# multimodallearning/DG-TTA

Measured on AMD Instinct MI355X. Metric: TTA-epochs/sec per GPU on 128^3 patch; Dice delta vs reference, higher is better.
Workload: dtype fp16

## Files before the change

### dg_tta_amd/_lib.py

```python
import ctypes as C
import os
from pathlib import Path

LIB_PATH = Path(__file__).resolve().parent / "libdgtta_hip.so"

_c_float_p = C.POINTER(C.c_float)
P, I, I64, U64, F, SZ = C.c_void_p, C.c_int, C.c_int64, C.c_uint64, C.c_float, C.c_size_t

SIGNATURES = {
    "dgtta_version": (I, []),
    "dgtta_last_error": (C.c_char_p, []),
    "dgtta_reload_env": (I, []),
    "dgtta_mind3d_ws_bytes": (SZ, [I, I, I, I]),
    "dgtta_mind3d_fwd": (I, [P, P, F, I, C.POINTER(F), I, P, I, I, I, P, SZ, I, I, I, I, P]),
    "dgtta_mind3d_noise_fill": (I, [P, U64, U64, I, I, I, I, I, P]),
    "dgtta_mind3d_fwd_seeded": (I, [P, U64, U64, I, F, I, C.POINTER(F), I, P, I, I, I, P, SZ, I, I, I, I, P]),
    "dgtta_gin_ws_bytes": (SZ, [I, I, I, I]),
    "dgtta_gin_chain_fwd": (I, [P, P, C.POINTER(I), C.POINTER(P), C.POINTER(P), P, P, SZ, I, I, I, I, P]),
    "dgtta_affine_warp3d_fwd": (I, [P, P, P, I, I, I, I, I, I, I, I, I, I, I, I, I, I, P, P]),
    "dgtta_affine_warp3d_bwd": (I, [P, P, P, I, I, I, I, I, I, I, I, I, I, I, I, I, P]),
    "dgtta_rf_field_ws_bytes": (SZ, [I, I, I, I]),
    "dgtta_rf_field_fwd": (I, [P, P, P, SZ, I, I, I, I, I, I, I, I, P]),
    "dgtta_diffeo_fields_ws_bytes": (SZ, [I, I, I, I]),
    "dgtta_diffeo_fields": (I, [P, F, P, P, P, SZ, I, I, I, I, I, P]),
# ... 47 lines not shown
    "dgtta_conv3d_kwgrad_ws_bytes": (SZ, [I, I, I, I, I, I, I, I, I, I]),
    "dgtta_conv3d_wgrad": (I, [P, I, P, I, P, P, P, SZ, I, I, I, I, I, I, I, I, I, I, I, I, P]),
    "dgtta_convT3d_s_fwd_ws_bytes": (SZ, [I, I, I, I, I, I]),
    "dgtta_convT3d_s_fwd": (I, [P, I, P, P, P, I, P, SZ, I, I, I, I, I, I, I, I, I, I, P]),
    "dgtta_convT3d_s_bwd_ws_bytes": (SZ, [I, I, I, I, I, I, I, I, I]),
    "dgtta_convT3d_s_bwd": (I, [P, I, P, I, P, P, I, P, P, P, SZ, I, I, I, I, I, I, I, I, I, I, I, P]),
    "dgtta_seghead_fwd": (I, [P, I, P, P, P, I, P, I, I, I, I, I64, I, P]),
    "dgtta_seghead_bwd_ws_bytes": (SZ, [I, I, I, I64]),
    "dgtta_seghead_bwd": (I, [P, I, P, I, P, P, I, P, I, P, P, P, SZ, I, I, I64, I, I, P]),
    "dgtta_seghead_bwd_acc": (I, [P, I, P, I, P, P, I, P, I, P, P, P, SZ, I, I, I64, I, I, I, P]),
    "dgtta_seghead_warp_supported": (I, [P, I, I, I, I, I, I, I]),
    "dgtta_seghead_warp_bwd_ws_bytes": (SZ, [I, I, I, I, I, I]),
    "dgtta_seghead_warp_fwd": (I, [P, P, P, P, I, P, P, I, I, I, I, I, I, I, P]),
    "dgtta_seghead_warp_bwd": (I, [P, P, P, P, P, P, I, P, P, P, P, SZ, I, I, I, I, I, I, I, I, P]),
    "dgtta_seghead_warp_bwd_g16": (I, [P, P, P, P, P, P, I, P, P, P, P, SZ, I, I, I, I, I, I, I, I, P]),
    "dgtta_ncdhw_to_ndhwc": (I, [P, P, I, I, I64, I, I, P]),
    "dgtta_ndhwc_to_ncdhw": (I, [P, P, I, I, I64, I, I, P]),
    "dgtta_argmax_dice": (I, [P, I, I, P, P, P, I, I64, P]),
    "dgtta_resample_axis_ws_bytes": (SZ, [I64, I, I64, I]),
    "dgtta_resample_axis": (I, [P, P, P, SZ, I64, I, I, I64, I, P]),
    "dgtta_window_accumulate": (I, [P, P, P, P, I, I, I, I, I, I, I, I, I, I, P]),
    "dgtta_seghead_window_accumulate": (I, [P, P, P, P, P, P, I, I, I, I, I, I, I, I, I, I, I, I, P]),
    "dgtta_logits_chunk_f64": (I, [P, P, P, I, I, I, I, I, I, I, I, I, I, I, I, P]),
    "dgtta_window_accumulate_t": (I, [P, P, P, P, I, I, I, I, I, I, I, I, I, I, I, P]),
    "dgtta_seghead_window_accumulate_t": (I, [P, P, P, P, P, P, I, I, I, I, I, I, I, I, I, I, I, I, I, P]),
    "dgtta_argmax_rows": (I, [P, I, I, I64, P, P]),
    "dgtta_feature_window_accumulate": (I, [P, P, P, P, I, I, I, I, I, I, I, I, I, I, I, P]),
    "dgtta_feature_window_accumulate_norm": (I, [P, P, P, P, F, P, P, P, I, I, I, I, I, I, I, I, I, I, I, P]),
    "dgtta_feature_window_accumulate_multi": (I, [P, P, P, I, P, P, F, P, P, P, I, I, I, I, I, I, I, I, I, I, I, I, P]),
    "dgtta_feature_head_argmax": (I, [P, I64, P, P, P, I, I, I, I64, P, P]),
# ... 103 lines not shown
```

### dg_tta_amd/csrc/conv_api.h

```cpp
#pragma once
#include "common.h"

static inline bool dtype_ok(int dtype) { return dtype == DGTTA_F32 || dtype == DGTTA_BF16 || dtype == DGTTA_F16; }
static inline size_t esize(int dtype) { return dtype == DGTTA_F32 ? 4 : 2; }

static inline int conv_granule(int dtype) { return dtype == DGTTA_F32 ? 8 : 16; }
static inline size_t n32(int c) { return (size_t)(c + 31) / 32 * 32; }

static inline int out_dim(int i, int s, int k = 3) { return (i + 2 * (k / 2) - k) / s + 1; }

static inline int gs_blocks(int64_t total, int cap = 16384) {
  int64_t b = (total + 255) / 256;
  return (int)(b < cap ? (b > 0 ? b : 1) : cap);
}

static inline int reduce_blocks(int64_t V, int B) {
  int64_t b = cdiv64(V, 32);
  int64_t cap = 4096 / (B > 0 ? B : 1);
  if (cap < 128) cap = 128;
  if (cap > 2048) cap = 2048;
  return (int)(b < cap ? (b > 0 ? b : 1) : cap);
}

struct ConvProblem {
// ... 65 lines not shown

int conv3_wgrad_mfma(const ConvProblem &P, Src x, Src dy, float *dw_t, Region ws, int accumulate);
size_t conv3_wgrad_mfma_ws_bytes(int B, int Cin, int Cout, int D, int H, int W);
size_t conv3_wgrad_split_extra_bytes(int B, int Cin, int Cout, int D, int H, int W, int stride);
bool conv3_wgrad_blocked_ok(const ConvProblem &P);
size_t conva_wgrad_ws_bytes(int B, int Cin, int Cout, int D, int H, int W);
int conva_wgrad_mfma(const ConvProblem &P, Src x, Src dy, float *dw_t, Region ws, int accumulate);

int convT_wgrad_mfma(const ConvProblem &P, Src x, Src dout, float *dw_t, Region ws, int accumulate, Region bias_part, int *bias_units);
int convT_bias_finalize(const float *part, int units, int Cout, float *db, int accumulate, hipStream_t st);
size_t convT_wgrad_split_extra_bytes(int B, int Cin, int Cout, int Di, int Hi, int Wi);
int convTa_wgrad_mfma(const ConvProblem &P, Src x, Src dout, float *dw_t, Region ws, int accumulate);

size_t head_wgrad_mfma_ws_bytes(int Cin, int nsel, int64_t rows);
int head_wgrad_mfma(const void *x, int ldx, const float *dout, int lddo, float *dw_sel, void *ws, size_t ws_bytes, int Cin,
                    int nsel, int64_t rows, int accumulate, int dtype, hipStream_t st, bool have_d16);

int head_fwd_mfma(const void *x, int ldx, const float *w, const float *bias, const int *sel, int nsel, float *out, int ldo, int Cin,
                  int64_t rows, int dtype, hipStream_t st);
int head_dgrad_mfma(const float *dout, int lddo, const float *w, const int *sel, int nsel, void *dx, int lddx, int Cin, int64_t rows,
                    int accumulate_dx, int dtype, hipStream_t st);
int head_wgrad_rows_mfma(const void *x, int ldx, const float *dout, int lddo, float *part, int nsplit, int nsel, int Cin, int64_t rows,
                         int dtype, hipStream_t st);

int conv3_pack_weights_ref(const ConvProblem &P, const float *w_t, void *wf, void *wb);
int conv3_fwd_ref(const ConvProblem &P, Src x, const void *wf, const float *bias, Dst y);
int conv3_dgrad_ref(const ConvProblem &P, Src dy, const void *wb, Dst dx, int accumulate);
int conv3_wgrad_ref(const ConvProblem &P, Src x, Src dy, float *part, int nsplit, float *dw_t, int accumulate);
int convT_fwd_ref(const ConvProblem &P, Src x, const float *w_t, const float *bias, Dst out);
int convT_dgrad_ref(const ConvProblem &P, Src dout, const float *w_t, Dst dx);
int convT_wgrad_ref(const ConvProblem &P, Src x, Src dout, float *part, int nsplit, float *dw_t, int accumulate);
// ... 35 lines not shown
```

### dg_tta_amd/csrc/head_wgrad.hip

```cpp
#include "conv_wgrad_common.h"

namespace {
template <typename T16>
__global__ void f32_to_16_rows_kernel(const float *__restrict__ src, int lds_, unsigned short *__restrict__ dst, int C,
                                      int64_t rows) {
  const int64_t n = rows * C;
  for (int64_t i = (int64_t)blockIdx.x * blockDim.x + threadIdx.x; i < n; i += (int64_t)gridDim.x * blockDim.x)
    dst[i] = f32_to_16<T16>(src[(i / C) * lds_ + i % C]);
}
}

struct PWG {
  static constexpr int CHUNK = 128, NBUF = 4, LA = 2;
  static constexpr int X_B = CHUNK * 64, BUF_B = 2 * X_B;
  static constexpr int LDS_BYTES = NBUF * BUF_B;
};

template <typename T16>
__global__ __launch_bounds__(256, 2) void pointwise_wgrad_kernel(const bf16_t *__restrict__ x, int ldx,
                                                                 const unsigned short *__restrict__ d16, int nsel,
                                                                 float *__restrict__ partial, int64_t nchunks) {
  extern __shared__ __attribute__((aligned(16))) unsigned char smem[];
  const int tid = threadIdx.x, lane = tid & 63;
  const int wave = __builtin_amdgcn_readfirstlane(tid >> 6);
// ... 59 lines not shown
      if (g + j < G) s += v[j];
  }
  if (k < nsel && c < Cin) {
    float *o = dw + (int64_t)k * Cin + c;
    *o = accumulate ? *o + s : s;
  }
}

size_t head_wgrad_mfma_ws_bytes(int Cin, int nsel, int64_t rows) {
  if (rows <= 0 || rows % 128 || rows / 128 >= (1ll << 30)) return 0;
  const int D = (int)(rows / 128);
  return conv3_wgrad_mfma_ws_bytes(1, Cin, nsel, D, 4, 32) + align_up((size_t)rows * nsel * 2, 256);
}

int head_wgrad_mfma(const void *x, int ldx, const float *dout, int lddo, float *dw_sel, void *ws, size_t ws_bytes, int Cin,
                    int nsel, int64_t rows, int accumulate, int dtype, hipStream_t st, bool have_d16) {
  if (rows % 128 || rows / 128 >= (1ll << 30)) return DGTTA_ERR_UNSUPPORTED;
  const int D = (int)(rows / 128);
  if (ws_bytes < head_wgrad_mfma_ws_bytes(Cin, nsel, rows)) return DGTTA_ERR_UNSUPPORTED;
  Taps real;
  for (int t = 0; t < 27; ++t) real.wt[t] = -1;
  real.wt[13] = 0;
  RealTaps reals;
  const WgradClasses wc = wgrad_single_class(1u << 13, real, &reals);
  const WgradOut out{dw_sel, Cin, 1, 0, accumulate};
  WgradLaunch L{x, dense_view(1, D, 4, 32, ldx), dout, dense_view(1, D, 4, 32, lddo), 1, Cin, nsel, dtype, ws, ws_bytes, st};
  if (dtype == DGTTA_F32) return wgrad_launch_classes(L, out, wc, reals);
  if (dtype == DGTTA_BF16 || dtype == DGTTA_F16) {
    const size_t cbytes = align_up((size_t)rows * nsel * 2, 256);
    unsigned short *d16 = (unsigned short *)ws;
    if (!have_d16) {
      if (dtype == DGTTA_BF16)
        hipLaunchKernelGGL(f32_to_16_rows_kernel<bf16_t>, dim3(2048), dim3(256), 0, st, dout, lddo, d16, nsel, rows);
      else
        hipLaunchKernelGGL(f32_to_16_rows_kernel<f16_t>, dim3(2048), dim3(256), 0, st, dout, lddo, d16, nsel, rows);
      DG_CHECK_LAUNCH("f32_to_16_rows_kernel");
    }
    const int G = 512;
    if (Cin == 32 && ldx >= 32 && ldx % 8 == 0 && nsel % 8 == 0 && nsel <= 32 && !((uintptr_t)x & 15) &&
        ws_bytes - cbytes >= (size_t)G * 1024 * sizeof(float) && dgtta_switches().wgrad_tr != '0') {
      float *partial = reinterpret_cast<float *>((char *)ws + cbytes);
      const int64_t nchunks = rows / PWG::CHUNK;
      const int g = (int)(nchunks < G ? nchunks : G);
      static DynLdsOnce once_b, once_h;
      if (dtype == DGTTA_BF16) {
// ... 23 lines not shown
```

### dg_tta_amd/csrc/instnorm.hip

```cpp
#include "conv_api.h"
#include "gfx950.h"

namespace {

template <typename T, int MODE>
__global__ __launch_bounds__(256) void chan_reduce_kernel(const T *__restrict__ y, int ldy, const T *__restrict__ gz,
                                                          int ldgz, const float *__restrict__ mean_rstd,
                                                          const float *__restrict__ gamma,
                                                          const float *__restrict__ beta, float slope,
                                                          double *__restrict__ partial, int C, int64_t V) {
  __shared__ float red[2][256];
  const int b = blockIdx.y;
  int CL = 1;
  while (CL < C && CL < 64) CL <<= 1;
  const int RG = 256 / CL;
  const int cl = threadIdx.x % CL, rg = threadIdx.x / CL;
  const int64_t rows_per_blk = cdiv64(V, gridDim.x);
  const int64_t r0 = (int64_t)blockIdx.x * rows_per_blk, r1 = (r0 + rows_per_blk < V) ? r0 + rows_per_blk : V;
  for (int c0 = 0; c0 < C; c0 += CL) {
    const int c = c0 + cl;
    float s0 = 0.f, s1 = 0.f;
    if (c < C) {
      float mu = 0.f, rs = 0.f, ga = 0.f, be = 0.f;
      if (MODE == 1) {
// ... 370 lines not shown
    float g = ld_f<T>(gz + row * ldgz + c);
    g = a > 0.f ? g : g * slope;
    st_f<T>(dy + row * lddy + c, (ga * rs) * ((g - c12[bc * 2]) - xh * c12[bc * 2 + 1]));
  }
}

__global__ void bias_finalize_kernel(const double *__restrict__ partial, int nblk, int B, int C, float *__restrict__ db,
                                     int accumulate) {
  const int c = blockIdx.x;
  double s = 0.0;
  for (int k = threadIdx.x; k < B * nblk; k += 64) s += partial[(((int64_t)k * C) + c) * 2];
  s = wave_sum_d(s);
  if (threadIdx.x == 0) db[c] = accumulate ? db[c] + (float)s : (float)s;
}

}

__global__ void set_header_kernel(long long *hdr, long long v) { hdr[0] = v; }

int conv_stats_ref(const void *y, int ldy, void *stats, int B, int C, int64_t V, int dtype, hipStream_t st) {
  const int nblk = reduce_blocks(V, B);
  hipLaunchKernelGGL(set_header_kernel, dim3(1), dim3(1), 0, st, (long long *)stats, (long long)nblk);
  DISPATCH_T(dtype, hipLaunchKernelGGL((chan_reduce_kernel<T, 0>), dim3(nblk, B), dim3(256), 0, st, (const T *)y, ldy,
                                       (const T *)nullptr, 0, nullptr, nullptr, nullptr, 0.f, (double *)stats + 32,
                                       C, V));
  DG_CHECK_LAUNCH("chan_reduce_kernel<0>");
  return DGTTA_OK;
}

size_t conv_bias_grad_ws_bytes(int B, int C, int64_t V) {
// ... 99 lines not shown
                                        float *dbeta, void *ws, size_t ws_bytes, int B, int C, int64_t V, float slope,
                                        int accumulate, int dtype, void *stream) {
  return instnorm_bwd_impl(gz, ldgz, y, ldy, gamma, beta, mean_rstd, dy, lddy, dgamma, dbeta, nullptr, ws, ws_bytes, B, C, V,
                           slope, accumulate, dtype, stream, "instnorm_lrelu_bwd");
}

extern "C" int dgtta_instnorm_lrelu_bwd_gstats(const void *gz, int ldgz, const void *y, int ldy, const float *gamma,
                                               const float *beta, const float *mean_rstd, void *dy, int lddy,
                                               float *dgamma, float *dbeta, const void *gstats, void *ws, size_t ws_bytes,
                                               int B, int C, int64_t V, float slope, int accumulate, int dtype,
                                               void *stream) {
  DG_REQUIRE(gstats, DGTTA_ERR_BADARG, "instnorm_lrelu_bwd_gstats: null statistics");
  return instnorm_bwd_impl(gz, ldgz, y, ldy, gamma, beta, mean_rstd, dy, lddy, dgamma, dbeta, gstats, ws, ws_bytes, B, C, V,
                           slope, accumulate, dtype, stream, "instnorm_lrelu_bwd_gstats");
}
```

### dg_tta_amd/csrc/warp.hip

```cpp
#include "conv_api.h"
#include "gfx950.h"
#include "sampler.h"
#include <limits.h>

namespace {


__device__ __forceinline__ Sample sample_from_base(const float *th, float x, float y, float z, int Ds, int Hs, int Ws,
                                                   int algebra, int pad_mode);

__device__ __forceinline__ Sample sample_pos(const float *th, int d, int h, int w, int Dd, int Hd, int Wd, int Ds,
                                             int Hs, int Ws, int algebra, int pad_mode) {
  return sample_from_base(th, base_coord(w, Wd), base_coord(h, Hd), base_coord(d, Dd), Ds, Hs, Ws, algebra, pad_mode);
}

__device__ __forceinline__ Sample sample_from_base(const float *th, float x, float y, float z, int Ds, int Hs, int Ws,
                                                   int algebra, int pad_mode) {
  float gx = __builtin_fmaf(th[2], z, __builtin_fmaf(th[1], y, th[0] * x)) + th[3];
  float gy = __builtin_fmaf(th[6], z, __builtin_fmaf(th[5], y, th[4] * x)) + th[7];
  float gz = __builtin_fmaf(th[10], z, __builtin_fmaf(th[9], y, th[8] * x)) + th[11];
  if (algebra) {
    gx = (gx - x) + x;
    gy = (gy - y) + y;
    gz = (gz - z) + z;
// ... 506 lines not shown
    }
    f32x4_t a0 = {0.f, 0.f, 0.f, 0.f}, a1 = {0.f, 0.f, 0.f, 0.f};
#pragma unroll
    for (int s = 0; s < 8; s += 2) {
      a0 = __builtin_amdgcn_mfma_f32_16x16x4f32(wa[s], zbl[s], a0, 0, 0, 0);
      a1 = __builtin_amdgcn_mfma_f32_16x16x4f32(wa[s + 1], zbl[s + 1], a1, 0, 0, 0);
    }
    if (live && 4 * g < nsel) {
      float *op = out + ((int64_t)b * V + ((int64_t)d * H + h) * W + wv) * nsel + 4 * g;
      *reinterpret_cast<float4 *>(op) = make_float4((a0[0] + a1[0]) + b4[0] * wsum, (a0[1] + a1[1]) + b4[1] * wsum,
                                                    (a0[2] + a1[2]) + b4[2] * wsum, (a0[3] + a1[3]) + b4[3] * wsum);
    }
  }
}

template <typename T, bool G16 = false>
__global__ __launch_bounds__(256, 6) void head_warp_bwd_kernel(const void *__restrict__ gdst_, const float *__restrict__ theta,
                                                            const float *__restrict__ w, const int *__restrict__ sel,
                                                            int nsel, T *__restrict__ gz, unsigned short *__restrict__ d16,
                                                            double *__restrict__ bias_partial, int D, int H, int W,
                                                            int algebra, int gx, int gy) {
  __shared__ float sw[HW_NS * HW_CIN];
  __shared__ InvMap s_im;
  __shared__ float sred[4][HW_NS];
  const float *gdst = (const float *)gdst_;
  const unsigned short *gdst16 = (const unsigned short *)gdst_;
  for (int i = threadIdx.x; i < HW_NS * HW_CIN; i += 256) {
    const int k = i / HW_CIN;
    sw[i] = k < nsel ? w[(int64_t)(sel ? sel[k] : k) * HW_CIN + i % HW_CIN] : 0.f;
  }
  const int64_t V = (int64_t)D * H * W;
  const int tilesZ = (D + 3) >> 2;
  const int tile = (int)blockIdx.x;
  const int bx = tile % gx, by = (tile / gx) % gy, bz = tile / (gx * gy);
  const int b = bz / tilesZ;
  const int x = bx * 16 + (threadIdx.x & 15), y = by * 4 + ((threadIdx.x >> 4) & 3), zc_ = (bz % tilesZ) * 4 + (threadIdx.x >> 6);
  const float *th = theta + b * 12;
  if (threadIdx.x == 0) s_im = inverse_map(th, D, H, W, D, H, W, algebra);
  __syncthreads();
  const InvMap im = s_im;
  float acc[HW_NS];
#pragma unroll
  for (int q = 0; q < HW_NS; ++q) acc[q] = 0.f;
  const bool inside = x < W && y < H && zc_ < D;
// ... 79 lines not shown
              }
            }
          }
        }
      }
    }
  }
  if (inside) {
    const int64_t u = (int64_t)b * V + ((int64_t)zc_ * H + y) * W + x;
    unsigned short *dp = d16 + u * nsel;
#pragma unroll
    for (int q = 0; q < HW_NS; q += 4)
      if (q < nsel) *reinterpret_cast<uint2 *>(dp + q) = make_uint2(pack2_16<T>(acc[q], acc[q + 1]), pack2_16<T>(acc[q + 2], acc[q + 3]));
    T *gp = gz + u * HW_CIN;
#pragma unroll
    for (int qt = 0; qt < 4; ++qt) {
      float o[8] = {0.f, 0.f, 0.f, 0.f, 0.f, 0.f, 0.f, 0.f};
#pragma unroll
      for (int k = 0; k < HW_NS; ++k) {
        const float4 w0 = *reinterpret_cast<const float4 *>(sw + k * HW_CIN + qt * 8);
        const float4 w1 = *reinterpret_cast<const float4 *>(sw + k * HW_CIN + qt * 8 + 4);
        o[0] = __builtin_fmaf(acc[k], w0.x, o[0]);
        o[1] = __builtin_fmaf(acc[k], w0.y, o[1]);
        o[2] = __builtin_fmaf(acc[k], w0.z, o[2]);
        o[3] = __builtin_fmaf(acc[k], w0.w, o[3]);
        o[4] = __builtin_fmaf(acc[k], w1.x, o[4]);
        o[5] = __builtin_fmaf(acc[k], w1.y, o[5]);
        o[6] = __builtin_fmaf(acc[k], w1.z, o[6]);
        o[7] = __builtin_fmaf(acc[k], w1.w, o[7]);
      }
      *reinterpret_cast<uint4 *>(reinterpret_cast<unsigned short *>(gp) + qt * 8) = pack16<T>(o);
// ... 209 lines not shown
      hipLaunchKernelGGL((head_warp_fwd_mfma_kernel<f16_t>), dim3((unsigned)nblk), dim3(256), 0, (hipStream_t)stream,
                         (const f16_t *)z, theta, w, bias, sel, nsel, out, D, H, W, tta_grid_algebra, gx, gy);
  } else if (dtype == DGTTA_BF16) {
    HWF_LAUNCH(bf16_t);
  } else {
    HWF_LAUNCH(f16_t);
  }
#undef HWF_LAUNCH
  DG_CHECK_LAUNCH("head_warp_fwd_kernel");
  return DGTTA_OK;
}

static int seghead_warp_bwd_impl(const void *z, const void *gout, int gout16, const float *theta, const float *h_theta,
                                 const float *w, const int *sel, int nsel, void *gz, float *dw_sel, float *db_sel, void *ws,
                                 size_t ws_bytes, int B, int Cin, int D, int H, int W, int tta_grid_algebra, int accumulate,
                                 int dtype, void *stream) {
  DG_REQUIRE(z && gout && theta && h_theta && w && gz && ws, DGTTA_ERR_BADARG, "seghead_warp_bwd: null pointer");
  DG_REQUIRE(B > 0 && B <= 16 && D > 0 && H > 0 && W > 0, DGTTA_ERR_BADARG, "seghead_warp_bwd: bad dims");
  DG_REQUIRE(head_warp_shape_ok(Cin, nsel, dtype), DGTTA_ERR_UNSUPPORTED, "seghead_warp_bwd: unsupported shape / dtype");
  DG_REQUIRE(!dw_sel || head_warp_wgrad_ok(nsel), DGTTA_ERR_UNSUPPORTED,
             "seghead_warp_bwd: the weight gradient needs 8 or 16 selected classes (nsel %d; use the unfused path)", nsel);
  DG_REQUIRE(((uintptr_t)gout & 15) == 0 && ((uintptr_t)gz & 15) == 0, DGTTA_ERR_BADARG, "seghead_warp_bwd: unaligned operand");
  const size_t need = dgtta_seghead_warp_bwd_ws_bytes(B, Cin, nsel, D, H, W);
  DG_REQUIRE(need > 0, DGTTA_ERR_UNSUPPORTED, "seghead_warp_bwd: voxel count must be a multiple of 128");
  DG_REQUIRE(ws_bytes >= need, DGTTA_ERR_WORKSPACE, "seghead_warp_bwd: workspace too small");
  for (int b = 0; b < B; ++b)
    DG_REQUIRE(host_map_ok(h_theta + 12 * b, D, H, W), DGTTA_ERR_UNSUPPORTED,
               "seghead_warp_bwd: sample %d's map is singular or strongly minifying (use the unfused path)", b);
  hipStream_t st = (hipStream_t)stream;
  const int64_t rows = (int64_t)B * D * H * W;
  double *bias_partial = (double *)ws;
  void *ws_main = (char *)ws + head_warp_bias_region(B, D, H, W);
  const size_t main_bytes = ws_bytes - head_warp_bias_region(B, D, H, W);
  unsigned short *d16 = (unsigned short *)ws_main;
  const int gx = cdiv(W, 16), gy = cdiv(H, 4);
  const int64_t nblk = (int64_t)gx * gy * cdiv(D, 4) * B;
  DG_REQUIRE(nblk < (1ll << 31), DGTTA_ERR_UNSUPPORTED, "seghead_warp_bwd: too many tiles");
#define HWB_LAUNCH(T, G)                                                                                            \
  hipLaunchKernelGGL((head_warp_bwd_kernel<T, G>), dim3((unsigned)nblk), dim3(256), 0, st, gout, theta, w, sel, nsel, \
                     (T *)gz, d16, db_sel ? bias_partial : nullptr, D, H, W, tta_grid_algebra, gx, gy)
  if (dtype == DGTTA_BF16) {
    if (gout16) HWB_LAUNCH(bf16_t, true);
    else HWB_LAUNCH(bf16_t, false);
  } else {
    if (gout16) HWB_LAUNCH(f16_t, true);
    else HWB_LAUNCH(f16_t, false);
  }
#undef HWB_LAUNCH
  DG_CHECK_LAUNCH("head_warp_bwd_kernel");
  if (dw_sel) {
    const int rc = head_wgrad_mfma(z, Cin, nullptr, nsel, dw_sel, ws_main, main_bytes, Cin, nsel, rows, accumulate, dtype, st, true);
    DG_REQUIRE(rc == DGTTA_OK, rc, "seghead_warp_bwd: head weight gradient failed (%d)", rc);
  }
  if (db_sel) {
    hipLaunchKernelGGL(head_warp_bias_finalize_kernel, dim3(HW_NS), dim3(1024), 0, st, bias_partial, (int)nblk, nsel, db_sel,
                       accumulate);
    DG_CHECK_LAUNCH("head_warp_bias_finalize_kernel");
  }
  return DGTTA_OK;
}

extern "C" int dgtta_seghead_warp_bwd(const void *z, const float *gout, const float *theta, const float *h_theta,
                                      const float *w, const int *sel, int nsel, void *gz, float *dw_sel, float *db_sel,
                                      void *ws, size_t ws_bytes, int B, int Cin, int D, int H, int W, int tta_grid_algebra,
                                      int accumulate, int dtype, void *stream) {
  return seghead_warp_bwd_impl(z, gout, 0, theta, h_theta, w, sel, nsel, gz, dw_sel, db_sel, ws, ws_bytes, B, Cin, D, H, W,
                               tta_grid_algebra, accumulate, dtype, stream);
}

extern "C" int dgtta_seghead_warp_bwd_g16(const void *z, const void *gout16, const float *theta, const float *h_theta,
                                          const float *w, const int *sel, int nsel, void *gz, float *dw_sel, float *db_sel,
                                          void *ws, size_t ws_bytes, int B, int Cin, int D, int H, int W, int tta_grid_algebra,
                                          int accumulate, int dtype, void *stream) {
  return seghead_warp_bwd_impl(z, gout16, 1, theta, h_theta, w, sel, nsel, gz, dw_sel, db_sel, ws, ws_bytes, B, Cin, D, H, W,
                               tta_grid_algebra, accumulate, dtype, stream);
}
```

### dg_tta_amd/unet_exec.py

```python
import collections
import contextlib
import ctypes as C
import os

import torch

from . import _lib
from ._lib import check, ptr, stream_of
from ._state import state_of
from .ops import F32, F16, _ws, dtype_code

EPS, SLOPE = 1e-5, 1e-2


def _wgrad_on_side_stream():
    return os.environ.get("DGTTA_WGRAD_STREAM", "1") != "0"


def _pad(c, m):
    return (c + m - 1) // m * m


def _k3(k):
    return tuple(k) if isinstance(k, (tuple, list)) else (k, k, k)
# ... 444 lines not shown
    D, H, W = dims
    cin = head.in_channels
    assert gz.ld >= cin and z.ld >= cin
    g = gout.contiguous(memory_format=torch.channels_last_3d).float()
    need_hw = head.weight.requires_grad or head.bias.requires_grad
    dws = p.empty(nsel, cin, dtype=torch.float32) if need_hw else None
    dbs = p.empty(nsel, dtype=torch.float32) if need_hw else None
    nb = p.lib.dgtta_seghead_bwd_ws_bytes(p.B, cin, nsel, D * H * W)
    ws = p.ws.get(nb)
    check(p.lib.dgtta_seghead_bwd_acc(z.ptr, z.ld, ptr(g), nsel, ptr(head.weight), ptr(sel), nsel, gz.ptr, gz.ld, ptr(dws), ptr(dbs),
                                      ptr(ws), nb, p.B, cin, D * H * W, 0, 1, p.dt, p.st), "dgtta_seghead_bwd_acc")
    if need_hw:
        _scatter_head_grads(p, head, sel, dws, dbs)


def _head_backward(p, head, z, sel, nsel, fw, g16, gout, dims):
    lib, B, dt, st = p.lib, p.B, p.dt, p.st
    D, H, W = dims
    if g16 is not None and any(gout.stride()):
        gout = gout + g16.permute(0, 4, 1, 2, 3).float()
        g16 = None
    g = None if g16 is not None else gout.contiguous(memory_format=torch.channels_last_3d).float()
    cin = head.in_channels
    gz = p.empty(B, D, H, W, cin)
    need_hw = head.weight.requires_grad or head.bias.requires_grad
    dws = p.empty(nsel, cin, dtype=torch.float32) if need_hw else None
    dbs = p.empty(nsel, dtype=torch.float32) if need_hw else None
    if fw is not None:
        nb = lib.dgtta_seghead_warp_bwd_ws_bytes(B, cin, nsel, D, H, W)
        ws = p.ws.get(nb)
        assert g16 is None or (tuple(g16.shape) == (B, D, H, W, nsel) and g16.dtype == p.adt and g16.is_contiguous())
        bwd = lib.dgtta_seghead_warp_bwd if g16 is None else lib.dgtta_seghead_warp_bwd_g16
        check(bwd(z.ptr, ptr(g if g16 is None else g16), ptr(fw[0]), ptr(fw[1]), ptr(head.weight), ptr(sel), nsel, ptr(gz),
                  ptr(dws), ptr(dbs), ptr(ws), nb, B, cin, D, H, W, 1, 0, dt, st), bwd.__name__)
    else:
        nb = lib.dgtta_seghead_bwd_ws_bytes(B, cin, nsel, D * H * W)
        ws = p.ws.get(nb)
        check(lib.dgtta_seghead_bwd(z.ptr, z.ld, ptr(g), nsel, ptr(head.weight), ptr(sel), nsel, ptr(gz), cin, ptr(dws), ptr(dbs),
                                    ptr(ws), nb, B, cin, D * H * W, 0, dt, st), "dgtta_seghead_bwd")
    if need_hw:
        _scatter_head_grads(p, head, sel, dws, dbs)
    return _Rows(gz, gz.data_ptr(), cin)


def _norm_backward(p, blk, gz, gstats):
    lib, B, cout, v = p.lib, p.B, blk.cout, blk.vout
    norm = blk.mod.norm
    dy = p.empty(B, *blk.dout, cout)
    nb = lib.dgtta_instnorm_ws_bytes(B, cout, v)
    ws = p.ws.get(nb)
    dgam = p.gbuf(norm.weight) if norm.weight.requires_grad else torch.empty_like(norm.weight)
    dbet = p.gbuf(norm.bias) if norm.bias.requires_grad else torch.empty_like(norm.bias)
    if gstats is not None:
        check(lib.dgtta_instnorm_lrelu_bwd_gstats(gz.ptr, gz.ld, ptr(blk.y), cout, ptr(norm.weight), ptr(norm.bias), ptr(blk.mr),
                                                  ptr(dy), cout, ptr(dgam), ptr(dbet), ptr(gstats), ptr(ws), nb, B, cout, v,
                                                  SLOPE, p.acc, p.dt, p.st), "dgtta_instnorm_lrelu_bwd_gstats")
    else:
        check(lib.dgtta_instnorm_lrelu_bwd(gz.ptr, gz.ld, ptr(blk.y), cout, ptr(norm.weight), ptr(norm.bias), ptr(blk.mr), ptr(dy),
                                           cout, ptr(dgam), ptr(dbet), ptr(ws), nb, B, cout, v, SLOPE, p.acc, p.dt, p.st),
              "dgtta_instnorm_lrelu_bwd")
    return dy


def _weight_grad(p, blk, dy):
    conv = blk.mod.conv
    if not (conv.weight.requires_grad or conv.bias.requires_grad):
        return
    nb = blk.wgrad_ws_bytes(p)
# ... 122 lines not shown
```

### include/dgtta.h

```cpp
#ifndef DGTTA_H
#define DGTTA_H

#include <stddef.h>
#include <stdint.h>

#ifdef __cplusplus
extern "C" {
#endif

#define DGTTA_OK 0
#define DGTTA_ERR_BADARG (-1)
#define DGTTA_ERR_UNSUPPORTED (-2)
#define DGTTA_ERR_WORKSPACE (-3)
#define DGTTA_ERR_LAUNCH (-4)

#define DGTTA_F32 0
#define DGTTA_BF16 1
#define DGTTA_F16 2

#define DGTTA_PAD_ZEROS 0
#define DGTTA_PAD_BORDER 1
#define DGTTA_INTERP_LINEAR 0
#define DGTTA_INTERP_NEAREST 1

// ... 111 lines not shown
                             float *mean_rstd, void *z, int ldz, void *ws, size_t ws_bytes, int B, int C,
                             int64_t V, float eps, float slope, int dtype, void *stream);
int dgtta_instnorm_lrelu_bwd(const void *gz, int ldgz, const void *y, int ldy, const float *gamma,
                             const float *beta, const float *mean_rstd, void *dy, int lddy, float *dgamma,
                             float *dbeta, void *ws, size_t ws_bytes, int B, int C, int64_t V, float slope,
                             int accumulate, int dtype, void *stream);

int dgtta_conv3d_k3_dgrad_gstats(const void *dy, int lddy, const void *wpack, void *dx, int lddx, int B, int Cin, int Cout,
                                 int CinP, int CoutP, int Di, int Hi, int Wi, const void *y_prev, int ldy_prev,
                                 const float *mean_rstd_prev, const float *gamma_prev, const float *beta_prev, float slope,
                                 void *gstats, size_t gstats_bytes, int *h_produced, int dtype, int impl, void *stream);
int dgtta_instnorm_lrelu_bwd_gstats(const void *gz, int ldgz, const void *y, int ldy, const float *gamma, const float *beta,
                                    const float *mean_rstd, void *dy, int lddy, float *dgamma, float *dbeta,
                                    const void *gstats, void *ws, size_t ws_bytes, int B, int C, int64_t V, float slope,
                                    int accumulate, int dtype, void *stream);

size_t dgtta_convT3d_fwd_ws_bytes(int Cin, int Cout, int dtype);
int dgtta_convT3d_k2s2_fwd(const void *x, int ldx, const float *w_t, const float *bias, void *out, int ldo, void *ws,
                           size_t ws_bytes, int B, int Cin, int Cout, int Di, int Hi, int Wi, int dtype, int impl,
                           void *stream);
size_t dgtta_convT3d_bwd_ws_bytes(int B, int Cin, int Cout, int Di, int Hi, int Wi);
size_t dgtta_convT3d_bwd_split_ws_bytes(int B, int Cin, int Cout, int Di, int Hi, int Wi);
int dgtta_convT3d_k2s2_bwd(const void *x, int ldx, const void *dout, int lddo, const float *w_t, void *dx, int lddx,
                           float *dw_t, float *db, void *ws, size_t ws_bytes, int B, int Cin, int Cout, int Di,
                           int Hi, int Wi, int accumulate, int dtype, int impl, void *stream);

size_t dgtta_conv3d_kpacked_bytes(int kd, int CinP, int CoutP, int dtype);
int dgtta_conv3d_kpack_weights(const float *w_t, void *wpack, int kd, int kh, int kw, int Cin, int Cout, int CinP, int CoutP,
                               int dtype, void *stream);
int dgtta_conv3d_fwd(const void *x, int ldx, const void *wpack, const float *bias, void *y, int ldy, void *stats, int B, int Cin,
// ... 20 lines not shown
                      int B, int Cin, int64_t V, int accumulate, int dtype, void *stream);
int dgtta_seghead_bwd_acc(const void *x, int ldx, const float *dout, int lddo, const float *w, const int *sel,
                          int nsel, void *dx, int lddx, float *dw_sel, float *db_sel, void *ws, size_t ws_bytes,
                          int B, int Cin, int64_t V, int accumulate, int accumulate_dx, int dtype, void *stream);

int dgtta_seghead_warp_supported(const float *h_theta, int B, int Cin, int nsel, int D, int H, int W, int dtype);
size_t dgtta_seghead_warp_bwd_ws_bytes(int B, int Cin, int nsel, int D, int H, int W);
int dgtta_seghead_warp_fwd(const void *z, const float *w, const float *bias, const int *sel, int nsel, const float *theta,
                           float *out, int B, int Cin, int D, int H, int W, int tta_grid_algebra, int dtype, void *stream);
int dgtta_seghead_warp_bwd(const void *z, const float *gout, const float *theta, const float *h_theta, const float *w,
                           const int *sel, int nsel, void *gz, float *dw_sel, float *db_sel, void *ws, size_t ws_bytes, int B,
                           int Cin, int D, int H, int W, int tta_grid_algebra, int accumulate, int dtype, void *stream);
int dgtta_seghead_warp_bwd_g16(const void *z, const void *gout16, const float *theta, const float *h_theta, const float *w,
                               const int *sel, int nsel, void *gz, float *dw_sel, float *db_sel, void *ws, size_t ws_bytes, int B,
                               int Cin, int D, int H, int W, int tta_grid_algebra, int accumulate, int dtype, void *stream);

int dgtta_ncdhw_to_ndhwc(const float *src, void *dst, int B, int C, int64_t V, int ldc, int dtype, void *stream);
int dgtta_ndhwc_to_ncdhw(const void *src, float *dst, int B, int C, int64_t V, int ldc, int dtype, void *stream);

int dgtta_argmax_dice(const float *logits, int ldc, int C, const int64_t *labels, int64_t *argmax_out,
                      int64_t *counts, int B, int64_t V, void *stream);

int dgtta_window_accumulate(const float *patch, const float *gauss, float *acc, float *nsum, int C, int PD, int PH,
                            int PW, int X, int Y, int Z, int x0, int y0, int z0, void *stream);

int dgtta_seghead_window_accumulate(const void *z, const float *w, const float *bias, const float *gauss, float *acc,
                                    float *nsum, int Cin, int C, int PD, int PH, int PW, int X, int Y, int Z, int x0, int y0,
                                    int z0, int dtype, void *stream);

int dgtta_window_accumulate_t(const float *patch, const float *gauss, void *acc, float *nsum, int C, int PD, int PH, int PW,
// ... 124 lines not shown
```

Baseline: 6.581.

## Fold segmentation-head input-gradient GEMM into instance-norm LReLU backward

When the head backward runs through the warped g16 path with 16 classes and 32 channels, it now writes only the 16-channel 16-bit class gradient instead of materialising the 32-channel gz tensor. A new instnorm backward kernel recomputes gz on the fly from that class gradient and the head weights using small MFMA ops, in both its statistics pass and its apply pass. This cuts the gz write and re-read traffic and drops the gz loop in the warp kernel, at the cost of doing the head matmul twice inside the norm backward. The path is on by default and can be disabled with an environment variable.

```diff
diff --git a/dg_tta_amd/_lib.py b/dg_tta_amd/_lib.py
--- a/dg_tta_amd/_lib.py
+++ b/dg_tta_amd/_lib.py
@@ -85,6 +85,8 @@
     "dgtta_seghead_warp_fwd": (I, [P, P, P, P, I, P, P, I, I, I, I, I, I, I, P]),
     "dgtta_seghead_warp_bwd": (I, [P, P, P, P, P, P, I, P, P, P, P, SZ, I, I, I, I, I, I, I, I, P]),
     "dgtta_seghead_warp_bwd_g16": (I, [P, P, P, P, P, P, I, P, P, P, P, SZ, I, I, I, I, I, I, I, I, P]),
+    "dgtta_seghead_warp_bwd_g16_d16": (I, [P, P, P, P, I, P, P, P, P, SZ, I, I, I, I, I, I, I, I, P]),
+    "dgtta_instnorm_lrelu_bwd_head": (I, [P, P, P, I, P, I, P, P, P, P, I, P, P, P, SZ, I, I, I64, F, I, I, P]),
     "dgtta_ncdhw_to_ndhwc": (I, [P, P, I, I, I64, I, I, P]),
     "dgtta_ndhwc_to_ncdhw": (I, [P, P, I, I, I64, I, I, P]),
     "dgtta_argmax_dice": (I, [P, I, I, P, P, P, I, I64, P]),
diff --git a/dg_tta_amd/csrc/conv_api.h b/dg_tta_amd/csrc/conv_api.h
--- a/dg_tta_amd/csrc/conv_api.h
+++ b/dg_tta_amd/csrc/conv_api.h
@@ -103,7 +103,8 @@
 
 size_t head_wgrad_mfma_ws_bytes(int Cin, int nsel, int64_t rows);
 int head_wgrad_mfma(const void *x, int ldx, const float *dout, int lddo, float *dw_sel, void *ws, size_t ws_bytes, int Cin,
-                    int nsel, int64_t rows, int accumulate, int dtype, hipStream_t st, bool have_d16);
+                    int nsel, int64_t rows, int accumulate, int dtype, hipStream_t st, bool have_d16,
+                    const unsigned short *d16_ext = nullptr);
 
 int head_fwd_mfma(const void *x, int ldx, const float *w, const float *bias, const int *sel, int nsel, float *out, int ldo, int Cin,
                   int64_t rows, int dtype, hipStream_t st);
diff --git a/dg_tta_amd/csrc/head_wgrad.hip b/dg_tta_amd/csrc/head_wgrad.hip
--- a/dg_tta_amd/csrc/head_wgrad.hip
+++ b/dg_tta_amd/csrc/head_wgrad.hip
@@ -97,7 +97,8 @@
 }
 
 int head_wgrad_mfma(const void *x, int ldx, const float *dout, int lddo, float *dw_sel, void *ws, size_t ws_bytes, int Cin,
-                    int nsel, int64_t rows, int accumulate, int dtype, hipStream_t st, bool have_d16) {
+                    int nsel, int64_t rows, int accumulate, int dtype, hipStream_t st, bool have_d16,
+                    const unsigned short *d16_ext) {
   if (rows % 128 || rows / 128 >= (1ll << 30)) return DGTTA_ERR_UNSUPPORTED;
   const int D = (int)(rows / 128);
   if (ws_bytes < head_wgrad_mfma_ws_bytes(Cin, nsel, rows)) return DGTTA_ERR_UNSUPPORTED;
@@ -111,7 +112,7 @@
   if (dtype == DGTTA_F32) return wgrad_launch_classes(L, out, wc, reals);
   if (dtype == DGTTA_BF16 || dtype == DGTTA_F16) {
     const size_t cbytes = align_up((size_t)rows * nsel * 2, 256);
-    unsigned short *d16 = (unsigned short *)ws;
+    unsigned short *d16 = have_d16 && d16_ext ? const_cast<unsigned short *>(d16_ext) : (unsigned short *)ws;
     if (!have_d16) {
       if (dtype == DGTTA_BF16)
         hipLaunchKernelGGL(f32_to_16_rows_kernel<bf16_t>, dim3(2048), dim3(256), 0, st, dout, lddo, d16, nsel, rows);
diff --git a/dg_tta_amd/csrc/instnorm.hip b/dg_tta_amd/csrc/instnorm.hip
--- a/dg_tta_amd/csrc/instnorm.hip
+++ b/dg_tta_amd/csrc/instnorm.hip
@@ -408,6 +408,126 @@
   if (threadIdx.x == 0) db[c] = accumulate ? db[c] + (float)s : (float)s;
 }
 
+constexpr int INH_C = 32, INH_NS = 16;
+
+__device__ __forceinline__ uint2 ld8_nt(const void *p) {
+  typedef __attribute__((ext_vector_type(2))) unsigned u32x2_t;
+  const u32x2_t v = __builtin_nontemporal_load(reinterpret_cast<const u32x2_t *>(p));
+  return make_uint2(v[0], v[1]);
+}
+
+template <typename T, int APPLY>
+__global__ __launch_bounds__(256) void in_bwd_head_kernel(const T *__restrict__ y, int ldy, const unsigned short *__restrict__ d16,
+                                                          const float *__restrict__ w, const int *__restrict__ sel,
+                                                          const float *__restrict__ mean_rstd, const float *__restrict__ gamma,
+                                                          const float *__restrict__ beta, const float *__restrict__ c12,
+                                                          float slope, double *__restrict__ partial, T *__restrict__ dy,
+                                                          int lddy, int64_t V, int nt) {
+  __shared__ float sred[APPLY ? 1 : 64 * INH_C * 2];
+  const int b = blockIdx.y;
+  const int lane = threadIdx.x & 63, wave = threadIdx.x >> 6;
+  const int n = lane & 15, g = lane >> 4;
+  float wa0[4], wa1[4];
+  {
+    const int ch = 8 * (n >> 2) + (n & 3);
+#pragma unroll
+    for (int s = 0; s < 4; ++s) {
+      const int k = 4 * g + s;
+      const float *wr = w + (int64_t)(sel ? sel[k] : k) * INH_C + ch;
+      wa0[s] = wr[0];
+      wa1[s] = wr[4];
+    }
+  }
+  float mu[8], rs[8], ga[8], be[8], k1[8], k2[8], s0[8], s1[8];
+#pragma unroll
+  for (int e = 0; e < 8; ++e) {
+    const int c = 8 * g + e;
+    mu[e] = mean_rstd[((int64_t)b * INH_C + c) * 2];
+    rs[e] = mean_rstd[((int64_t)b * INH_C + c) * 2 + 1];
+    ga[e] = gamma[c];
+    be[e] = beta[c];
+    k1[e] = APPLY ? c12[((int64_t)b * INH_C + c) * 2] : 0.f;
+    k2[e] = APPLY ? c12[((int64_t)b * INH_C + c) * 2 + 1] : 0.f;
+    s0[e] = s1[e] = 0.f;
+  }
+  const T *yb = y + (int64_t)b * V * ldy + 8 * g;
+  const unsigned short *db = d16 + (int64_t)b * V * INH_NS + 4 * g;
+  T *ob = APPLY ? dy + (int64_t)b * V * lddy + 8 * g : nullptr;
+  auto gz_of = [&](const uint2 &dv, float *gz) {
+    float d[4];
+    unpack2_16<T>(dv.x, d[0], d[1]);
+    unpack2_16<T>(dv.y, d[2], d[3]);
+    f32x4_t a0 = {0.f, 0.f, 0.f, 0.f}, a1 = {0.f, 0.f, 0.f, 0.f};
+#pragma unroll
+    for (int s = 0; s < 4; ++s) {
+      a0 = __builtin_amdgcn_mfma_f32_16x16x4f32(wa0[s], d[s], a0, 0, 0, 0);
+      a1 = __builtin_amdgcn_mfma_f32_16x16x4f32(wa1[s], d[s], a1, 0, 0, 0);
+    }
+#pragma unroll
+    for (int e = 0; e < 4; ++e) gz[e] = a0[e], gz[4 + e] = a1[e];
+  };
+  auto one = [&](const uint4 &yv, const uint2 &dv, int64_t row) {
+    float f[8], gz[8], o[8];
+    unpack16<T>(yv, f);
+    gz_of(dv, gz);
+    if (row >= V) return;
+#pragma unroll
+    for (int e = 0; e < 8; ++e) {
+      const float xh = (f[e] - mu[e]) * rs[e];
+      const float a = xh * ga[e] + be[e];
+      const float gg = a > 0.f ? gz[e] : gz[e] * slope;
+      if (APPLY) {
+        o[e] = (ga[e] * rs[e]) * ((gg - k1[e]) - xh * k2[e]);
+      } else {
+        s0[e] += gg;
+        s1[e] += gg * xh;
+      }
+    }
+    if (APPLY) {
+      const uint4 pk = pack16<T>(o);
+      if (nt) st16_nt(ob + row * lddy, pk);
+      else *reinterpret_cast<uint4 *>(ob + row * lddy) = pk;
+    }
+  };
+  const int64_t ustep = (int64_t)gridDim.x * 4;
+  for (int64_t u = (int64_t)blockIdx.x * 4 + wave; u * 16 < V; u += 2 * ustep) {
+    const int64_t r0 = u * 16 + n, r1 = (u + ustep) * 16 + n;
+    const bool two = (u + ustep) * 16 < V;
+    const uint4 zero4 = make_uint4(0, 0, 0, 0);
+    const uint2 zero2 = make_uint2(0, 0);
+    uint4 y0 = zero4, y1 = zero4;
+    uint2 d0 = zero2, d1 = zero2;
+    if (r0 < V) {
+      y0 = ld16_nt(yb + r0 * ldy);
+      d0 = ld8_nt(db + r0 * INH_NS);
+    }
+    if (two && r1 < V) {
+      y1 = ld16_nt(yb + r1 * ldy);
+      d1 = ld8_nt(db + r1 * INH_NS);
+    }
+    one(y0, d0, r0);
+    if (two) one(y1, d1, r1);
+  }
+  if (APPLY) return;
+#pragma unroll
+  for (int e = 0; e < 8; ++e) {
+    sred[((wave * 16 + n) * INH_C + 8 * g + e) * 2 + 0] = s0[e];
+    sred[((wave * 16 + n) * INH_C + 8 * g + e) * 2 + 1] = s1[e];
+  }
+  __syncthreads();
+  if (threadIdx.x < INH_C) {
+    const int c = threadIdx.x;
+    double t0 = 0.0, t1 = 0.0;
+    for (int k = 0; k < 64; ++k) {
+      t0 += (double)sred[(k * INH_C + c) * 2];
+      t1 += (double)sred[(k * INH_C + c) * 2 + 1];
+    }
+    double *p = partial + ((((int64_t)b * gridDim.x + blockIdx.x) * INH_C) + c) * 2;
+    p[0] = t0;
+    p[1] = t1;
+  }
+}
+
 }
 
 __global__ void set_header_kernel(long long *hdr, long long v) { hdr[0] = v; }
@@ -537,3 +657,43 @@
   return instnorm_bwd_impl(gz, ldgz, y, ldy, gamma, beta, mean_rstd, dy, lddy, dgamma, dbeta, gstats, ws, ws_bytes, B, C, V,
                            slope, accumulate, dtype, stream, "instnorm_lrelu_bwd_gstats");
 }
+
+extern "C" int dgtta_instnorm_lrelu_bwd_head(const void *d16, const float *w, const int *sel, int nsel, const void *y, int ldy,
+                                             const float *gamma, const float *beta, const float *mean_rstd, void *dy, int lddy,
+                                             float *dgamma, float *dbeta, void *ws, size_t ws_bytes, int B, int C, int64_t V,
+                                             float slope, int accumulate, int dtype, void *stream) {
+  DG_REQUIRE(d16 && w && y && gamma && beta && mean_rstd && dy && dgamma && dbeta && ws, DGTTA_ERR_BADARG,
+             "instnorm_lrelu_bwd_head: null pointer");
+  DG_REQUIRE(B > 0 && V > 0 && ldy >= C && lddy >= C, DGTTA_ERR_BADARG, "instnorm_lrelu_bwd_head: bad dims");
+  DG_REQUIRE(C == INH_C && nsel == INH_NS && (dtype == DGTTA_BF16 || dtype == DGTTA_F16), DGTTA_ERR_UNSUPPORTED,
+             "instnorm_lrelu_bwd_head: built for 32 channels, 16 selected classes and 16-bit storage (C %d, nsel %d, dtype %d)", C,
+             nsel, dtype);
+  DG_REQUIRE(ldy % 8 == 0 && lddy % 8 == 0 && !((uintptr_t)y & 15) && !((uintptr_t)dy & 15) && !((uintptr_t)d16 & 15),
+             DGTTA_ERR_BADARG, "instnorm_lrelu_bwd_head: unaligned operand");
+  DG_REQUIRE(ws_bytes >= dgtta_instnorm_ws_bytes(B, C, V), DGTTA_ERR_WORKSPACE, "instnorm_lrelu_bwd_head: workspace too small");
+  hipStream_t st = (hipStream_t)stream;
+  const int nblk = reduce_blocks(V, B);
+  double *partial = (double *)ws;
+  float *c12 = (float *)((char *)ws + align_up((size_t)B * nblk * C * 2 * sizeof(double), 256));
+  const int64_t units = cdiv64(V, 16);
+  const int blocks = (int)(cdiv64(units, 4 * 4) < 4096 ? cdiv64(units, 4 * 4) : 4096);
+  const int nt = dgtta_switches().in_nt - '0';
+#define INH_LAUNCH(T)                                                                                                         \
+  do {                                                                                                                        \
+    hipLaunchKernelGGL((in_bwd_head_kernel<T, 0>), dim3(nblk, B), dim3(256), 0, st, (const T *)y, ldy,                        \
+                       (const unsigned short *)d16, w, sel, mean_rstd, gamma, beta, (const float *)nullptr, slope, partial,  \
+                       (T *)nullptr, 0, V, nt);                                                                               \
+    DG_CHECK_LAUNCH("in_bwd_head_kernel<0>");                                                                                 \
+    hipLaunchKernelGGL(in_bwd_finalize_kernel, dim3(C), dim3(256), 0, st, partial, nblk, B, C, V, c12, dgamma, dbeta,         \
+                       accumulate);                                                                                           \
+    DG_CHECK_LAUNCH("in_bwd_finalize_kernel");                                                                                \
+    hipLaunchKernelGGL((in_bwd_head_kernel<T, 1>), dim3(blocks, B), dim3(256), 0, st, (const T *)y, ldy,                      \
+                       (const unsigned short *)d16, w, sel, mean_rstd, gamma, beta, (const float *)c12, slope,               \
+                       (double *)nullptr, (T *)dy, lddy, V, nt);                                                              \
+    DG_CHECK_LAUNCH("in_bwd_head_kernel<1>");                                                                                 \
+  } while (0)
+  if (dtype == DGTTA_BF16) INH_LAUNCH(bf16_t);
+  else INH_LAUNCH(f16_t);
+#undef INH_LAUNCH
+  return DGTTA_OK;
+}
diff --git a/dg_tta_amd/csrc/warp.hip b/dg_tta_amd/csrc/warp.hip
--- a/dg_tta_amd/csrc/warp.hip
+++ b/dg_tta_amd/csrc/warp.hip
@@ -544,7 +544,7 @@
   }
 }
 
-template <typename T, bool G16 = false>
+template <typename T, bool G16 = false, bool GZ = true>
 __global__ __launch_bounds__(256, 6) void head_warp_bwd_kernel(const void *__restrict__ gdst_, const float *__restrict__ theta,
                                                             const float *__restrict__ w, const int *__restrict__ sel,
                                                             int nsel, T *__restrict__ gz, unsigned short *__restrict__ d16,
@@ -555,9 +555,11 @@
   __shared__ float sred[4][HW_NS];
   const float *gdst = (const float *)gdst_;
   const unsigned short *gdst16 = (const unsigned short *)gdst_;
-  for (int i = threadIdx.x; i < HW_NS * HW_CIN; i += 256) {
-    const int k = i / HW_CIN;
-    sw[i] = k < nsel ? w[(int64_t)(sel ? sel[k] : k) * HW_CIN + i % HW_CIN] : 0.f;
+  if (GZ) {
+    for (int i = threadIdx.x; i < HW_NS * HW_CIN; i += 256) {
+      const int k = i / HW_CIN;
+      sw[i] = k < nsel ? w[(int64_t)(sel ? sel[k] : k) * HW_CIN + i % HW_CIN] : 0.f;
+    }
   }
   const int64_t V = (int64_t)D * H * W;
   const int tilesZ = (D + 3) >> 2;
@@ -667,7 +669,7 @@
       if (q < nsel) *reinterpret_cast<uint2 *>(dp + q) = make_uint2(pack2_16<T>(acc[q], acc[q + 1]), pack2_16<T>(acc[q + 2], acc[q + 3]));
     T *gp = gz + u * HW_CIN;
 #pragma unroll
-    for (int qt = 0; qt < 4; ++qt) {
+    for (int qt = 0; GZ && qt < 4; ++qt) {
       float o[8] = {0.f, 0.f, 0.f, 0.f, 0.f, 0.f, 0.f, 0.f};
 #pragma unroll
       for (int k = 0; k < HW_NS; ++k) {
@@ -907,8 +909,9 @@
 static int seghead_warp_bwd_impl(const void *z, const void *gout, int gout16, const float *theta, const float *h_theta,
                                  const float *w, const int *sel, int nsel, void *gz, float *dw_sel, float *db_sel, void *ws,
                                  size_t ws_bytes, int B, int Cin, int D, int H, int W, int tta_grid_algebra, int accumulate,
-                                 int dtype, void *stream) {
-  DG_REQUIRE(z && gout && theta && h_theta && w && gz && ws, DGTTA_ERR_BADARG, "seghead_warp_bwd: null pointer");
+                                 int dtype, void *stream, void *d16_out = nullptr) {
+  DG_REQUIRE(z && gout && theta && h_theta && ws && (d16_out || (w && gz)), DGTTA_ERR_BADARG, "seghead_warp_bwd: null pointer");
+  if (d16_out) gz = d16_out;
   DG_REQUIRE(B > 0 && B <= 16 && D > 0 && H > 0 && W > 0, DGTTA_ERR_BADARG, "seghead_warp_bwd: bad dims");
   DG_REQUIRE(head_warp_shape_ok(Cin, nsel, dtype), DGTTA_ERR_UNSUPPORTED, "seghead_warp_bwd: unsupported shape / dtype");
   DG_REQUIRE(!dw_sel || head_warp_wgrad_ok(nsel), DGTTA_ERR_UNSUPPORTED,
@@ -925,24 +928,28 @@
   double *bias_partial = (double *)ws;
   void *ws_main = (char *)ws + head_warp_bias_region(B, D, H, W);
   const size_t main_bytes = ws_bytes - head_warp_bias_region(B, D, H, W);
-  unsigned short *d16 = (unsigned short *)ws_main;
+  unsigned short *d16 = d16_out ? (unsigned short *)d16_out : (unsigned short *)ws_main;
   const int gx = cdiv(W, 16), gy = cdiv(H, 4);
   const int64_t nblk = (int64_t)gx * gy * cdiv(D, 4) * B;
   DG_REQUIRE(nblk < (1ll << 31), DGTTA_ERR_UNSUPPORTED, "seghead_warp_bwd: too many tiles");
-#define HWB_LAUNCH(T, G)                                                                                            \
-  hipLaunchKernelGGL((head_warp_bwd_kernel<T, G>), dim3((unsigned)nblk), dim3(256), 0, st, gout, theta, w, sel, nsel, \
+#define HWB_LAUNCH(T, G, GZ)                                                                                            \
+  hipLaunchKernelGGL((head_warp_bwd_kernel<T, G, GZ>), dim3((unsigned)nblk), dim3(256), 0, st, gout, theta, w, sel, nsel, \
                      (T *)gz, d16, db_sel ? bias_partial : nullptr, D, H, W, tta_grid_algebra, gx, gy)
-  if (dtype == DGTTA_BF16) {
-    if (gout16) HWB_LAUNCH(bf16_t, true);
-    else HWB_LAUNCH(bf16_t, false);
+  if (d16_out) {
+    if (dtype == DGTTA_BF16) HWB_LAUNCH(bf16_t, true, false);
+    else HWB_LAUNCH(f16_t, true, false);
+  } else if (dtype == DGTTA_BF16) {
+    if (gout16) HWB_LAUNCH(bf16_t, true, true);
+    else HWB_LAUNCH(bf16_t, false, true);
   } else {
-    if (gout16) HWB_LAUNCH(f16_t, true);
-    else HWB_LAUNCH(f16_t, false);
+    if (gout16) HWB_LAUNCH(f16_t, true, true);
+    else HWB_LAUNCH(f16_t, false, true);
   }
 #undef HWB_LAUNCH
   DG_CHECK_LAUNCH("head_warp_bwd_kernel");
   if (dw_sel) {
-    const int rc = head_wgrad_mfma(z, Cin, nullptr, nsel, dw_sel, ws_main, main_bytes, Cin, nsel, rows, accumulate, dtype, st, true);
+    const int rc = head_wgrad_mfma(z, Cin, nullptr, nsel, dw_sel, ws_main, main_bytes, Cin, nsel, rows, accumulate, dtype, st, true,
+                                   d16_out ? d16 : nullptr);
     DG_REQUIRE(rc == DGTTA_OK, rc, "seghead_warp_bwd: head weight gradient failed (%d)", rc);
   }
   if (db_sel) {
@@ -968,3 +975,12 @@
   return seghead_warp_bwd_impl(z, gout16, 1, theta, h_theta, w, sel, nsel, gz, dw_sel, db_sel, ws, ws_bytes, B, Cin, D, H, W,
                                tta_grid_algebra, accumulate, dtype, stream);
 }
+
+extern "C" int dgtta_seghead_warp_bwd_g16_d16(const void *z, const void *gout16, const float *theta, const float *h_theta,
+                                              int nsel, void *d16_out, float *dw_sel, float *db_sel, void *ws, size_t ws_bytes,
+                                              int B, int Cin, int D, int H, int W, int tta_grid_algebra, int accumulate, int dtype,
+                                              void *stream) {
+  DG_REQUIRE(d16_out, DGTTA_ERR_BADARG, "seghead_warp_bwd_g16_d16: null pointer");
+  return seghead_warp_bwd_impl(z, gout16, 1, theta, h_theta, nullptr, nullptr, nsel, nullptr, dw_sel, db_sel, ws, ws_bytes, B, Cin,
+                               D, H, W, tta_grid_algebra, accumulate, dtype, stream, d16_out);
+}
diff --git a/dg_tta_amd/unet_exec.py b/dg_tta_amd/unet_exec.py
--- a/dg_tta_amd/unet_exec.py
+++ b/dg_tta_amd/unet_exec.py
@@ -482,6 +482,9 @@
         _scatter_head_grads(p, head, sel, dws, dbs)
 
 
+_HeadGrad = collections.namedtuple("_HeadGrad", "d16 head sel nsel")
+
+
 def _head_backward(p, head, z, sel, nsel, fw, g16, gout, dims):
     lib, B, dt, st = p.lib, p.B, p.dt, p.st
     D, H, W = dims
@@ -490,10 +493,21 @@
         g16 = None
     g = None if g16 is not None else gout.contiguous(memory_format=torch.channels_last_3d).float()
     cin = head.in_channels
-    gz = p.empty(B, D, H, W, cin)
     need_hw = head.weight.requires_grad or head.bias.requires_grad
     dws = p.empty(nsel, cin, dtype=torch.float32) if need_hw else None
     dbs = p.empty(nsel, dtype=torch.float32) if need_hw else None
+    if (fw is not None and g16 is not None and nsel == 16 and cin == 32 and z.ld == 32 and p.esz == 2 and p.impl != 1
+            and os.environ.get("DGTTA_HEAD_GZ_FOLD", "1") != "0"):
+        nb = lib.dgtta_seghead_warp_bwd_ws_bytes(B, cin, nsel, D, H, W)
+        ws = p.ws.get(nb)
+        assert tuple(g16.shape) == (B, D, H, W, nsel) and g16.dtype == p.adt and g16.is_contiguous()
+        d16 = p.empty(B, D, H, W, nsel)
+        check(lib.dgtta_seghead_warp_bwd_g16_d16(z.ptr, ptr(g16), ptr(fw[0]), ptr(fw[1]), nsel, ptr(d16), ptr(dws), ptr(dbs), ptr(ws),
+                                                 nb, B, cin, D, H, W, 1, 0, dt, st), "dgtta_seghead_warp_bwd_g16_d16")
+        if need_hw:
+            _scatter_head_grads(p, head, sel, dws, dbs)
+        return _HeadGrad(d16, head, sel, nsel)
+    gz = p.empty(B, D, H, W, cin)
     if fw is not None:
         nb = lib.dgtta_seghead_warp_bwd_ws_bytes(B, cin, nsel, D, H, W)
         ws = p.ws.get(nb)
@@ -519,7 +533,12 @@
     ws = p.ws.get(nb)
     dgam = p.gbuf(norm.weight) if norm.weight.requires_grad else torch.empty_like(norm.weight)
     dbet = p.gbuf(norm.bias) if norm.bias.requires_grad else torch.empty_like(norm.bias)
-    if gstats is not None:
+    if isinstance(gz, _HeadGrad):
+        assert cout == 32 and gstats is None
+        check(lib.dgtta_instnorm_lrelu_bwd_head(ptr(gz.d16), ptr(gz.head.weight), ptr(gz.sel), gz.nsel, ptr(blk.y), cout,
+                                                ptr(norm.weight), ptr(norm.bias), ptr(blk.mr), ptr(dy), cout, ptr(dgam), ptr(dbet),
+                                                ptr(ws), nb, B, cout, v, SLOPE, p.acc, p.dt, p.st), "dgtta_instnorm_lrelu_bwd_head")
+    elif gstats is not None:
         check(lib.dgtta_instnorm_lrelu_bwd_gstats(gz.ptr, gz.ld, ptr(blk.y), cout, ptr(norm.weight), ptr(norm.bias), ptr(blk.mr),
                                                   ptr(dy), cout, ptr(dgam), ptr(dbet), ptr(gstats), ptr(ws), nb, B, cout, v,
                                                   SLOPE, p.acc, p.dt, p.st), "dgtta_instnorm_lrelu_bwd_gstats")
diff --git a/include/dgtta.h b/include/dgtta.h
--- a/include/dgtta.h
+++ b/include/dgtta.h
@@ -149,6 +149,10 @@
                                     const float *mean_rstd, void *dy, int lddy, float *dgamma, float *dbeta,
                                     const void *gstats, void *ws, size_t ws_bytes, int B, int C, int64_t V, float slope,
                                     int accumulate, int dtype, void *stream);
+int dgtta_instnorm_lrelu_bwd_head(const void *d16, const float *w, const int *sel, int nsel, const void *y, int ldy,
+                                  const float *gamma, const float *beta, const float *mean_rstd, void *dy, int lddy,
+                                  float *dgamma, float *dbeta, void *ws, size_t ws_bytes, int B, int C, int64_t V, float slope,
+                                  int accumulate, int dtype, void *stream);
 
 size_t dgtta_convT3d_fwd_ws_bytes(int Cin, int Cout, int dtype);
 int dgtta_convT3d_k2s2_fwd(const void *x, int ldx, const float *w_t, const float *bias, void *out, int ldo, void *ws,
@@ -199,6 +203,9 @@
 int dgtta_seghead_warp_bwd_g16(const void *z, const void *gout16, const float *theta, const float *h_theta, const float *w,
                                const int *sel, int nsel, void *gz, float *dw_sel, float *db_sel, void *ws, size_t ws_bytes, int B,
                                int Cin, int D, int H, int W, int tta_grid_algebra, int accumulate, int dtype, void *stream);
+int dgtta_seghead_warp_bwd_g16_d16(const void *z, const void *gout16, const float *theta, const float *h_theta, int nsel,
+                                   void *d16_out, float *dw_sel, float *db_sel, void *ws, size_t ws_bytes, int B, int Cin, int D,
+                                   int H, int W, int tta_grid_algebra, int accumulate, int dtype, void *stream);
 
 int dgtta_ncdhw_to_ndhwc(const float *src, void *dst, int B, int C, int64_t V, int ldc, int dtype, void *stream);
 int dgtta_ndhwc_to_ncdhw(const void *src, float *dst, int B, int C, int64_t V, int ldc, int dtype, void *stream);
```

Result: faster. 6.679 (median of 6 runs) (+1.5%).
